# retrojetpacks/Gadget-Leicester

Hardware: AMD Instinct MI355X
Metric: particle-steps/sec (gravity+SPH) (higher is better)
Workload: dtype f64

## Files before the change

### gadget-leicester_amd/csrc/ghip_gravity.hip

```cpp
#include <cmath>

#include <hipcub/hipcub.hpp>

#include "ghip_walk.h"

__global__ void k_grav_finish(int nt, const int *__restrict__ tgt, const int *__restrict__ perm,
                              int n, double G, double comoving_fac, const double *__restrict__ pos,
                              const double *__restrict__ gravpm, double *__restrict__ oacc,
                              double *__restrict__ oldacc)
{
  int ti = blockIdx.x * blockDim.x + threadIdx.x;
  if(ti >= nt)
    return;
  int i = perm[tgt[ti]];
  double a0 = oacc[i], a1 = oacc[(size_t) n + i], a2 = oacc[2 * (size_t) n + i];
  if(comoving_fac != 0)
    {
      a0 += comoving_fac * pos[i];
      a1 += comoving_fac * pos[(size_t) n + i];
      a2 += comoving_fac * pos[2 * (size_t) n + i];
    }
  double b0 = a0, b1 = a1, b2 = a2;
  if(gravpm)
    {
// ... 537 lines not shown
{
  int per;
  ghip_shard_range(nt, ctx->shard_n, ctx->shard_rank, lo, cnt, &per);
}

struct WalkJob
{
  int walk;
  GravK k;
  WalkSeg sg;
  WalkPlan plan;
  PartialBufs pb;
  int nbuckets;
  unsigned long long *counter;
};

static int prepare_job(ghip_ctx *ctx, const ghip_grav_params *p, int walk, int nt, int slot,
                       WalkJob &J, hipStream_t plan_on = nullptr)
{
  hipStream_t ps = plan_on ? plan_on : ctx->stream;
  J.walk = walk;
  GCHK(prepare_tables(ctx, p, walk, J.k));
  walk_layout(ctx->dyn_use ? ctx->dyn.tree : ctx->gt, nt, J.sg, &J.nbuckets, walk == GHIP_WALK_EWALD);
  GCHK(build_plan(ctx, walk == GHIP_WALK_EWALD ? 1 : 0, J.nbuckets, J.sg.ns, J.plan, slot, ps));
  GCHK(ensure_partials(ctx, J.plan.nwaves, slot, J.pb));
  J.counter = ghip_cslot(ctx, walk == GHIP_WALK_EWALD ? GHIP_CK_EWALD : GHIP_CK_NEWTON);
  HIPCHK(hipMemsetAsync(J.counter, 0, GHIP_CKIND_U64 * 8, ps));
  return GHIP_OK;
}

static int run_walk(ghip_ctx *ctx, const WalkJob &J, int nt, const int *tgt, hipStream_t st)
{
  int evi = (J.walk == GHIP_WALK_EWALD) ? 4 : 2;
  ctx->plan_writer[J.walk == GHIP_WALK_EWALD ? 1 : 0] = st;
  HIPCHK(hipEventRecord(ctx->evp[evi], st));
  launch_walk_any(ctx, J.walk, ctx->dyn_use ? ctx->dyn.tree : ctx->gt, J.sg, J.nbuckets, nt, tgt, P<double>(ctx->sx),
                  P<double>(ctx->sy), P<double>(ctx->sz), P<double>(ctx->ssoft),
                  P<double>(ctx->soldacc), J.k, J.counter, J.plan, J.pb, st);
  HIPCHK(hipGetLastError());
  HIPCHK(hipEventRecord(ctx->evp[evi + 1], st));
  return GHIP_OK;
}

static int combine_walk(ghip_ctx *ctx, const WalkJob &J, int nt, const int *tgt, hipStream_t st)
{
  k_combine_grav<<<cdiv(nt, 256), 256, 0, st>>>(
    nt, J.plan, tgt, P<int>(ctx->gt.perm), J.pb.ax, J.pb.ay, J.pb.az, J.pb.cost, ctx->n,
    P<double>(ctx->f[GHIP_F_GRAVACCEL]), P<int>(ctx->f[GHIP_F_GRAVCOST]),
    J.walk == GHIP_WALK_EWALD ? 1 : 0, J.k.debug_steps);
  HIPCHK(hipGetLastError());
  return GHIP_OK;
}

static int pair_balance(ghip_ctx *ctx)
{
  if(!ctx->pc_ev[3][3])
    {
      for(int i = 0; i < 4; i++)
        for(int j = 0; j < 4; j++)
          if(!ctx->pc_ev[i][j])
            HIPCHK(hipEventCreate(&ctx->pc_ev[i][j]));
      return GHIP_OK;
    }
  for(int i = 0; i < 4; i++)
    {
      if(ctx->pc_cap[i] == 0)
        continue;
      hipEvent_t *e = ctx->pc_ev[i];
      if(hipEventQuery(e[1]) != hipSuccess || hipEventQuery(e[3]) != hipSuccess)
        {
          (void) hipGetLastError();
          continue;
        }
      float tn = 0, te = 0;
      if(hipEventElapsedTime(&tn, e[0], e[1]) == hipSuccess && hipEventElapsedTime(&te, e[2], e[3]) == hipSuccess)
        {
          const int k = ctx->pc_cap[i] > 8192 ? 1 : 0;
          const float fe = ctx->pc_hyd[i] ? 1.1f : 1.0f;
          const float c = tn > fe * te ? tn : fe * te;
          ctx->pc_cost[k] = c;
          ctx->pc_age[k] = 0;
        }
      else
        (void) hipGetLastError();
      ctx->pc_cap[i] = 0;
    }
  ctx->pc_age[0]++;
  ctx->pc_age[1]++;
  const int cur = ctx->pair_lds > 8192 ? 1 : 0, oth = cur ^ 1;
  if(ctx->pc_cost[cur] < 0)
    return GHIP_OK;
  int want = cur;
  const bool close = ctx->pc_cost[oth] > 0 && ctx->pc_cost[oth] < 1.1f * ctx->pc_cost[cur] &&
                     ctx->pc_cost[cur] < 1.1f * ctx->pc_cost[oth];
  if(ctx->pc_cost[oth] < 0 || ctx->pc_age[oth] > (close ? 16 : 64))
    want = oth;
  else if(ctx->pc_cost[oth] < ctx->pc_cost[cur])
    want = oth;
  ctx->pair_lds = want ? 10240 : 8192;
  static int dbg = -1;
  if(dbg < 0)
    dbg = getenv("GHIP_PAIR_DEBUG") ? 1 : 0;
  if(dbg)
    fprintf(stderr, "[pair_balance] cost 8K %.3f (age %d)  10K %.3f (age %d)  -> %d\n", ctx->pc_cost[0],
            ctx->pc_age[0], ctx->pc_cost[1], ctx->pc_age[1], ctx->pair_lds);
  return GHIP_OK;
}

int ghip_gravity_impl(ghip_ctx *ctx, const ghip_grav_params *p, int walk)
{
  if(!ctx->gt.built)
    return ghip_fail(ctx, GHIP_EINVAL, "ghip_gravity: call ghip_tree_build first");
  if(walk < 0 || walk > GHIP_WALK_NEWTON_EWALD)
    return ghip_fail(ctx, GHIP_EINVAL, "ghip_gravity: unknown walk %d", walk);
  const bool pair = (walk == GHIP_WALK_NEWTON_EWALD);
  if(pair && !p->periodic)
    return ghip_fail(ctx, GHIP_EINVAL, "ghip_gravity: the Newton+Ewald pair needs periodic = 1");
  if(ctx->tree_unverified)
    {
      ghip_ctx::GravCall c;
      c.p = *p;
      c.walk = walk;
      ctx->grav_log.push_back(c);
    }
  GCHK(ghip_build_target_lists(ctx));
  hipStream_t st = ctx->stream;
  int n = ctx->n;
  int lo, nt;
  shard_slice(ctx, ctx->nt_grav, &lo, &nt);
  ghip_stats &S = ctx->stats;
  if(walk == GHIP_WALK_EWALD || pair)
    S.ewald_interactions = 0;
  if(walk != GHIP_WALK_EWALD)
    {
      S.grav_interactions = 0;
      S.grav_targets = nt;
    }
  if(nt == 0 || n == 0)
    return GHIP_OK;
  const int *tgt = P<int>(ctx->tg_grav) + lo;
  WalkJob A, E;
  hipStream_t pn = (pair && ctx->plan_writer[0] == ctx->stream3) ? ctx->stream3 : nullptr;
  hipStream_t pe = (pair && ctx->plan_writer[1] == ctx->stream2) ? ctx->stream2 : nullptr;
  if(getenv("GHIP_PLAN_ON_MAIN"))
    pn = nullptr;
  GCHK(prepare_job(ctx, p, pair ? GHIP_WALK_NEWTON : walk, nt, 0, A, pn));
  if(pair)
    GCHK(prepare_job(ctx, p, GHIP_WALK_EWALD, nt, 1, E, pe));

  GCHK(ghip_gather_f64_lim(ctx, ctx->gt.n, P<int>(ctx->gt.perm), P<double>(ctx->f[GHIP_F_OLDACC]),
                           n, P<double>(ctx->soldacc)));
  if(!pair)
    {
      GCHK(run_walk(ctx, A, nt, tgt, st));
      return combine_walk(ctx, A, nt, tgt, st);
    }
  hipStream_t sN = ctx->stream3, sE = ctx->stream2;
  HIPCHK(hipEventRecord(ctx->evx[0], st));
// ... 220 lines not shown
```

### gadget-leicester_amd/csrc/ghip_internal.h

```cpp
#pragma once
#include <hip/hip_runtime.h>

#include <cstdint>
#include <cstdio>
#include <cstdlib>
#include <cstring>
#include <new>
#include <string>
#include <vector>

#include "../../include/ghip.h"
#include "ghip_count.h"

#define GHIP_BITS 21
#define GHIP_EN 64
#define GHIP_EW_NB ((GHIP_EN >> 1) + 1)
#define GHIP_EW_NKB (GHIP_EN / 3 + 1)
#define GHIP_EW_DOUBLES (GHIP_EW_NB * GHIP_EW_NB * GHIP_EW_NKB * 16)
static inline __host__ __device__ unsigned int ghip_ew_offset(int i, int j, int kb, int t)
{
  return (unsigned int) ((((i >> 1) * GHIP_EW_NB + (j >> 1)) * GHIP_EW_NKB + kb) * 16 +
                         ((i & 1) * 2 + (j & 1)) * 4 + t);
}
#define GHIP_NTAB 1000
// ... 172 lines not shown
  int du_sent = 0, du_recvd = 0;
  bool geom_kept = false;
  long long bytes_sent[16] = {0, 0, 0, 0, 0, 0, 0, 0, 0, 0, 0, 0, 0, 0, 0, 0};
  ghip_pm_params pm;
  DevBuf pm_all;
  int pmreg_grid = 0;
  ghip_pmnp_params pmnp;
  int pmnp_rc = 0;
  std::string pmnp_msg;
  ghip_pot_params pot;
  DevBuf pot_tgt;
  bool gt_is_pot = false;
  int pot_rc = 0;
  std::string pot_msg;
  ghip_dd_global_args gq;
  ghip_global_params gq_p;
  DevBuf gq_send, gq_all;
  ghip_dd_decomp_params dcp;
  DevBuf dc_own, dc_all;
  DevBuf dc_hist, dc_hist_all;
  int dc_level = 0, dc_bmax = 0, dc_shift = 0;
  int dc_rc = 0;
  std::string dc_msg;
  double dc_corner[3] = {0, 0, 0}, dc_center[3] = {0, 0, 0}, dc_len = 0;
};

static inline void ghip_dd_set_allgather(DDState &D, const void *send, size_t bytes, DevBuf *recv)
{
  D.x.kind = 1;
  D.x.send = send;
  D.x.bytes = bytes;
  D.x.recv = recv;
}

static inline void ghip_dd_set_alltoallv(DDState &D, const void *send, size_t recbytes,
                                         const int *scount, const int *soff, DevBuf *recv)
{
  D.x.kind = 2;
  D.x.send = send;
  D.x.bytes = recbytes;
  D.x.recv = recv;
  for(int r = 0; r < D.nranks; r++)
    {
      D.x.scount[r] = scount[r];
      D.x.soff[r] = soff[r];
    }
}

struct DevWords
{
  alignas(128) unsigned int pair_started;
  alignas(128) unsigned long long ghost_growth;
  unsigned long long timebin_hist[64];
  int sel_left;
  int list_count;
  int dust_partners;
  int gas_targets;
  int step_err;
  int pm_err;
  int tree_info[2][2];
};

struct alignas(64) PinnedWords
{
  TreeSizes sizes[2];
  int gas_mixed;
};

struct DynTree
{
  TreeDev tree;
  DevBuf ev, dp;
  DevBuf eh, cnt, fa;
  DevBuf kick;
  DevBuf kick_dv, kick_flag;
};

struct PmMesh
{
  int n = 0;
  void *fwd = nullptr, *inv = nullptr;
  DevBuf rho, k, force;
  struct Open
  {
    int n = 0;
    int table_n = 0;
    void *fwd = nullptr, *inv = nullptr;
    DevBuf rho, k, table, force, oct;
    Open() = default;
    Open(const Open &) = delete;
    Open &operator=(const Open &) = delete;
    ~Open();
  } open;
  PmMesh() = default;
  PmMesh(const PmMesh &) = delete;
  PmMesh &operator=(const PmMesh &) = delete;
  ~PmMesh();
};

struct ghip_ctx
{
  ghip_ctx() = default;
  ghip_ctx(const ghip_ctx &) = delete;
  ghip_ctx &operator=(const ghip_ctx &) = delete;
  ~ghip_ctx();

  int device = 0;
  hipStream_t stream = nullptr;
  std::string err;

  int n = 0, ngas = 0;
  DevBuf f[GHIP_F_COUNT];
  DevBuf stage, aosP, aosS;
  PinnedWords *pinned = nullptr;

  double corner[3] = {0, 0, 0}, center[3] = {0, 0, 0}, dlen = 0;
  double soft[6] = {0, 0, 0, 0, 0, 0};

  TreeDev gt;
  TreeDev st;
  DevBuf sx, sy, sz, ssoft, soldacc;
  DevBuf gp;
  DevBuf gq;
  DevBuf dleft, dright, drho, dnumngb, ddhsml, ddivv, drot, dflags, dtgt_a, dtgt_b, dhcur;
  DevBuf hpart;

  DevBuf act_host_idx;
  int nactive = -1;
  bool gas_mixed = false;
  int skip_massless = 0;
  bool massless_marked = false;
  bool gas_types_unknown = false;
  bool lists_dirty = true;
  bool gas_list_dirty = true;
  DevBuf tg_grav, tg_gas;
  int nt_grav = 0, nt_gas = 0;
  int shard_rank = 0, shard_n = 1;

  DevBuf tax, tay, taz, tcost;
  DevBuf tax2, tay2, taz2, tcost2, plan_nsub2, plan_woff2, plan_wave2, cubtmp2;
  hipStream_t stream2 = nullptr;
  hipStream_t stream3 = nullptr;
  bool adaptive_gravsoft = false;
  bool grav_pending = false;
  unsigned int *pair_started = nullptr;
  bool gas_pending = false;
  bool gas_wait_upload = false;
  hipEvent_t evx[4] = {};
  hipEvent_t evt[2] = {};
  DevBuf plan_steps[3][2], plan_nsub, plan_woff, plan_wave;
  int plan_nb[3] = {-1, -1, -1}, plan_ns[3] = {-1, -1, -1}, plan_cur[3] = {0, 0, 0};
// ... 1 lines not shown
  DevBuf cubtmp3;

  DevBuf ewtab;
  DevBuf ewbrick;
  double ew_box = 0;
  DevBuf srtab;
  bool srtab_ready = false;

  DevBuf cubtmp;
  PmMesh pm;
  ghip_pm_region pm_region = {};
  bool pm_region_set = false;
  DevBuf words;
  DevBuf cslots, rslots;
  ghip_stats stats;
  hipEvent_t ev[16] = {};
  DDState dd;
  DevBuf bh_swallow, bh_injected;
  DevBuf dust_heat;
  DevBuf dust_idx, dust_work, dust_pairs, dust_cub;
  DevBuf sfr_work, sfr_cub;
  int timestep_endrun = 0;
  bool iflags_on = false;
  ghip_integration_flags iflags = {};
  DevBuf kick_drag, kick_ddm, kick_newdens;
  bool has_drag = false, has_ddm = false, has_newdens = false;
  int kick_fields_n = -1, kick_fields_ngas = -1;

  bool visc_on = false;
  ghip_visc_params visc = {};
  DevBuf visc_alpha, visc_dtalpha;
  int visc_ngas = -1;
  long long visc_epoch = 0;

  bool async = false;
  bool tree_unverified = false;
  bool tree_async_ok = true;
  hipEvent_t ev_sizes = nullptr, ev_sizes_gas = nullptr;
  bool gas_unverified = false;
  bool gas_async = false;
  int build_gen = 0;
  bool sort_wide = false;
  bool in_recover = false;
  struct GravCall
  {
    ghip_grav_params p;
    int walk;
  };
  std::vector<GravCall> grav_log;
  std::vector<void *> host_pins;
  bool hydro_early = false;
  bool dyn_on = false, dyn_valid = false, dyn_use = false;
  DynTree dyn;
  int pair_lds = 10240;
  hipEvent_t pc_ev[4][4] = {};
  int pc_cap[4] = {0, 0, 0, 0};
  int pc_hyd[4] = {0, 0, 0, 0};
  int pc_head = 0;
  float pc_cost[2] = {-1.f, -1.f};
  int pc_age[2] = {0, 0};
  hipEvent_t ev_side = nullptr;

  std::vector<hipEvent_t> ev_ring;
  int ring_slots = 0, ring_cur = -1;
  hipEvent_t *evp = nullptr;
  long long run_steps = 0, run_syncs0 = 0, run_launches0 = 0, run_dens_iter = 0;
  long long n_syncs = 0;
  DevBuf pot;
  DevBuf pot_nint;
  int pot_n = -1;
  DevBuf potcorr;
  double potcorr_box = 0;
  DevBuf srpot;
  DevBuf gq_work;
};
#define GHIP_NEV 16

static inline hipError_t ghip_stream_sync(ghip_ctx *ctx, hipStream_t st)
{
  ctx->n_syncs++;
  return hipStreamSynchronize(st);
}
static inline hipError_t ghip_event_sync(ghip_ctx *ctx, hipEvent_t e)
{
  ctx->n_syncs++;
  return hipEventSynchronize(e);
}
long long ghip_launch_count(void);
int ghip_tree_verify(ghip_ctx *ctx);
int ghip_gas_verify(ghip_ctx *ctx);

int ghip_fail(ghip_ctx *ctx, int code, const char *fmt, ...);
#define GHIP_ERRW_PLAN 0
#define GHIP_ERRW_LET 1
#define GHIP_ERRW_TREE 2
#define GHIP_ERRW_PM 3
#define GHIP_ERRW_DRIFT 4
#define GHIP_ERRW_TIMESTEP 5
#define GHIP_ERRW_COUNT 8
int *ghip_errwords(void);
static inline int *ghip_errword(ghip_ctx *, int which) { return ghip_errwords() + which; }
int ghip_check_device_errors(ghip_ctx *ctx);
int ghip_join(ghip_ctx *ctx);
static inline int ghip_wg(const ghip_ctx *ctx) { return ctx->grav_pending ? 64 : 256; }
static inline int *ghip_gas_mixed_word(ghip_ctx *ctx) { return &ctx->pinned->gas_mixed; }
static inline DevWords *ghip_words(ghip_ctx *ctx) { return reinterpret_cast<DevWords *>(ctx->words.p); }
static inline unsigned long long *ghip_cslot(ghip_ctx *ctx, int kind)
{
  return reinterpret_cast<unsigned long long *>(ctx->cslots.p) + (size_t) kind * GHIP_CKIND_U64;
}
static inline unsigned long long *ghip_rslot(ghip_ctx *ctx, int kind)
{
  return reinterpret_cast<unsigned long long *>(ctx->rslots.p) + (size_t) kind * GHIP_CKIND_U64;
}
int ghip_read_slots(ghip_ctx *ctx, DevBuf &buf, unsigned long long out[GHIP_CK_COUNT][2]);
int ghip_mark_converted_gas(ghip_ctx *ctx);
int ghip_sink_buffers(ghip_ctx *ctx);
int ghip_unmark_massless_for_hydro(ghip_ctx *ctx);
int ghip_check_gas_types(ghip_ctx *ctx);
int ghip_dyn_capture(ghip_ctx *ctx);
int ghip_dyn_kick_recorded(ghip_ctx *ctx);
void ghip_dyn_release(ghip_ctx *ctx);
int ghip_fill_walk_records(ghip_ctx *ctx, TreeDev &t);
int ghip_gravity_finish_on(ghip_ctx *ctx, double G, int pmgrid, double comoving_fac, int all_shards,
                           hipStream_t st);
int ghip_join_pair(ghip_ctx *ctx);
int ghip_finish_gas_tree(ghip_ctx *ctx);
#define GHIP_JOIN(ctx)                          \
  do                                            \
    {                                           \
      int j_ = ghip_join(ctx);                  \
      if(j_ != GHIP_OK)                         \
        return j_;                              \
    }                                           \
  while(0)
void ghip_pm_release(ghip_ctx *ctx);
int ghip_pm_potential_add(ghip_ctx *ctx, const ghip_pm_params *p, double *pot);
int ghip_pm_potential_deposit(ghip_ctx *ctx, const ghip_pm_params *p);
int ghip_pm_potential_solve(ghip_ctx *ctx, const ghip_pm_params *p, int nranks, const double *all, double *pot);
int ghip_pmnp_potential_check(ghip_ctx *ctx, const ghip_grav_params *g, const ghip_pm_params *pm, const char *who);
int ghip_pmnp_potential_deposit(ghip_ctx *ctx, int pmgrid, int *outside);
int ghip_pmnp_potential_solve(ghip_ctx *ctx, int pmgrid, double G, int nranks, const double *all, double *pot);
size_t ghip_pmnp_block_bytes(int pmgrid);
const void *ghip_pmnp_block(ghip_ctx *ctx);
#define EXTENT_WORDS 16
int ghip_extent_pass(ghip_ctx *ctx, DevBuf &own, int use_work);
unsigned long long ghip_extent_reduce(const unsigned long long *all, int nranks, double xmin[3], double xmax[3],
                                      unsigned long long *ntot, int *bmin, int *bmax, int *bad);
#define EXTENT_ERR_POS 1ULL
#define EXTENT_ERR_WORK 2ULL
#define EXTENT_ERR_LOCAL 4ULL

#define HIPCHK(call)                                                                         \
  do                                                                                         \
    {                                                                                        \
      hipError_t e_ = (call);                                                                \
      if(e_ != hipSuccess)                                                                   \
// ... 123 lines not shown
```

### gadget-leicester_amd/csrc/ghip_sph.hip

```cpp

#include "ghip_ngb.h"
#include <cmath>

struct BucketBox
{
  double cx, cy, cz, ex, ey, ez, hmax;
};

__device__ __forceinline__ double d_first_lane_f64(double v)
{
  int lo = __builtin_amdgcn_readfirstlane(__double2loint(v));
  int hi = __builtin_amdgcn_readfirstlane(__double2hiint(v));
  return __hiloint2double(hi, lo);
}

__device__ __forceinline__ BucketBox d_bucket_box(bool valid, double px, double py, double pz,
                                                  double h, const BoxK b)
{
  BucketBox B;
  B.cx = d_first_lane_f64(px);
  B.cy = d_first_lane_f64(py);
  B.cz = d_first_lane_f64(pz);
  B.ex = d_wave_max_f64(valid ? fabs(d_wrap(px - B.cx, b)) : 0.0);
  B.ey = d_wave_max_f64(valid ? fabs(d_wrap(py - B.cy, b)) : 0.0);
// ... 541 lines not shown
      if(b < nblk)
        blockcnt[b] = run + incl - c;
      run += __shfl(incl, 63, 64);
    }
  if(threadIdx.x == 0)
    *total = run;
}

__global__ void __launch_bounds__(64) k_sel_scatter(int n, const int *__restrict__ in,
                                                    const int *__restrict__ flags,
                                                    const int *__restrict__ blockoff,
                                                    int *__restrict__ out)
{
  const int base = blockIdx.x * SEL_BLOCK;
  int off = blockoff[blockIdx.x];
  const unsigned long long below = (1ull << threadIdx.x) - 1ull;
  for(int j = 0; j < SEL_ITEMS; j++)
    {
      const int a = base + j * 64 + threadIdx.x;
      const bool keep = a < n && flags[a] != 0;
      const unsigned long long m = __ballot(keep);
      if(keep)
        out[off + __popcll(m & below)] = in[a];
      off += __popcll(m);
    }
}

int ghip_density_impl(ghip_ctx *ctx, const ghip_dens_params *p)
{
  GCHK(ghip_tree_verify(ctx));
  GCHK(ghip_finish_gas_tree(ctx));
  if(ctx->gas_wait_upload)
    return ghip_fail(ctx, GHIP_EINVAL, "ghip_density: ghip_upload_aos_particles was not followed by "
                     "ghip_upload_aos_gas");
  GCHK(ghip_gas_verify(ctx));
  if(!ctx->st.built)
    return ghip_fail(ctx, GHIP_EINVAL, "ghip_density: call ghip_tree_build first");
  GCHK(ghip_build_target_lists(ctx));
  ghip_stats &S = ctx->stats;
  S.dens_neighbours = 0;
  S.dens_target_evals = 0;
  S.dens_iterations = 0;
  int ng = ctx->ngas, n = ctx->n;
  int lo, nt;
  shard_slice(ctx, ctx->nt_gas, &lo, &nt);
  if(ng == 0 || nt == 0)
    return GHIP_OK;
  hipStream_t st = ctx->stream;
  TreeDev &t = ctx->st;
  GCHK(dens_alloc(ctx));
  double *hcur = P<double>(ctx->dhcur);
  unsigned long long *counter = ghip_cslot(ctx, GHIP_CK_DENS);
  unsigned long long *racc = ghip_rslot(ctx, GHIP_CK_DENS);
  int *dnum = &ghip_words(ctx)->sel_left;
  HIPCHK(hipMemsetAsync(counter, 0, GHIP_CKIND_U64 * 8, st));
  HIPCHK(hipEventRecord(ctx->evp[6], st));

  int *cur = P<int>(ctx->dtgt_a), *nxt = P<int>(ctx->dtgt_b);
  HIPCHK(hipMemcpyAsync(cur, P<int>(ctx->tg_gas) + lo, (size_t) nt * 4, hipMemcpyDeviceToDevice,
                        st));
  k_dens_init<<<cdiv(nt, ghip_wg(ctx)), ghip_wg(ctx), 0, st>>>(nt, cur, P<double>(ctx->gp), hcur,
                                             P<double>(ctx->dleft), P<double>(ctx->dright));
  BoxK b = make_box(p->BoxSize, p->periodic);
  DensFin F = {p->DesNumNgb, p->MaxNumNgbDeviation, p->MinGasHsml, p->Ti_Current,
               p->Timebase_interval};
  int maxiter = p->MaxIter > 0 ? p->MaxIter : 150;
  int ncur = nt, iter = 0;
  GCHK(ghip_ensure(ctx, ctx->cubtmp, ((size_t) cdiv(nt, SEL_BLOCK) + 2) * 4));
  int *seloff = P<int>(ctx->cubtmp);

  while(ncur > 0)
    {
      const int tgw = ghip_sph_tg();
      const int nbk = (ncur + tgw - 1) / tgw;
      int nsub = (ghip_sph_target_waves() + nbk - 1) / nbk;
      nsub = nsub < 1 ? 1 : (nsub > GHIP_MAXSUB ? GHIP_MAXSUB : nsub);
      SPH_LAUNCH(k_density, tgw, (nbk * nsub + 7) & ~7, st, P<TreeSizes>(t.dsz), P<SphNode>(t.mq), P<double>(ctx->gp), ncur,
                 nsub, cur, hcur, b, P<double>(ctx->drho), P<double>(ctx->dnumngb),
                 P<double>(ctx->ddhsml), P<double>(ctx->ddivv), P<double>(ctx->drot), counter, racc,
                 ghip_sph_xcd(), nbk * nsub);
      k_dens_finalize<<<cdiv(ncur, ghip_wg(ctx)), ghip_wg(ctx), 0, st>>>(
        ncur, nsub, cur, P<int>(t.perm), n, ng, F, P<double>(ctx->drho), P<double>(ctx->dnumngb),
        P<double>(ctx->ddhsml), P<double>(ctx->ddivv), P<double>(ctx->drot), hcur,
        P<double>(ctx->dleft), P<double>(ctx->dright), P<double>(ctx->f[GHIP_F_ENTROPY]),
        P<double>(ctx->f[GHIP_F_DTENTROPY]), P<int>(ctx->f[GHIP_F_TIMEBIN]),
        P<int>(ctx->f[GHIP_F_TI_BEGSTEP]), P<double>(ctx->gp), P<double>(ctx->gq),
        P<double>(ctx->f[GHIP_F_HSML]), P<double>(ctx->f[GHIP_F_NUMNGB]),
        P<double>(ctx->f[GHIP_F_DENSITY]), P<double>(ctx->f[GHIP_F_DHSMLFAC]),
        P<double>(ctx->f[GHIP_F_DIVVEL]), P<double>(ctx->f[GHIP_F_CURLVEL]),
        P<double>(ctx->f[GHIP_F_PRESSURE]), P<int>(ctx->dflags));
      HIPCHK(hipGetLastError());
      S.dens_target_evals += ncur;
      const int nblk = cdiv(ncur, SEL_BLOCK);
      k_sel_count<<<nblk, 64, 0, st>>>(ncur, P<int>(ctx->dflags), seloff);
      k_sel_scan<<<1, 64, 0, st>>>(nblk, seloff, dnum);
      int left = 0;
      HIPCHK(hipMemcpyAsync(&left, dnum, 4, hipMemcpyDeviceToHost, st));
      HIPCHK(ghip_stream_sync(ctx, st));
      GCHK(ghip_check_device_errors(ctx));
      if(left > 0)
        {
          k_sel_scatter<<<nblk, 64, 0, st>>>(ncur, cur, P<int>(ctx->dflags), seloff, nxt);
          HIPCHK(hipGetLastError());
        }
      ncur = left;
      int *tmp = cur;
      cur = nxt;
      nxt = tmp;
      if(ncur > 0)
        {
          iter++;
          if(iter > maxiter)
            return ghip_fail(ctx, GHIP_ENOCONV,
                             "density: %d particles not converged after %d h-iterations "
                             "(reference: endrun(1155), density.c:669-674)", ncur, maxiter);
        }
    }
  HIPCHK(hipEventRecord(ctx->evp[7], st));
  S.dens_iterations = iter;
  return GHIP_OK;
}

extern "C" int ghip_density(ghip_ctx *ctx, const ghip_dens_params *p)
{
  if(!ctx || !p)
    return GHIP_EINVAL;
  return ghip_density_impl(ctx, p);
}

extern "C" int ghip_update_hmax(ghip_ctx *ctx)
{
  if(!ctx)
    return GHIP_EINVAL;
  GCHK(ghip_tree_verify(ctx));
  GCHK(ghip_finish_gas_tree(ctx));
  GCHK(ghip_gas_verify(ctx));
  if(!ctx->st.built)
    return ghip_fail(ctx, GHIP_EINVAL, "ghip_update_hmax: no tree");
  return ghip_gastree_refresh_hmax(ctx);
}

extern "C" int ghip_density_evaluate(ghip_ctx *ctx, const ghip_dens_params *p, int target,
                                     double h, double out7[7])
{
  if(ctx)
    GHIP_JOIN(ctx);
  if(!ctx || !p || !out7)
    return GHIP_EINVAL;
  GCHK(ghip_finish_gas_tree(ctx));
  if(!ctx->st.built)
    return ghip_fail(ctx, GHIP_EINVAL, "ghip_density_evaluate: no tree");
// ... 698 lines not shown
```

### gadget-leicester_amd/csrc/ghip_tree.hip

```cpp
#include <hipcub/hipcub.hpp>

#include "ghip_internal.h"
#include "ghip_keys.h"

__global__ void k_morton_from_pos(int n, const double *__restrict__ x, const double *__restrict__ y,
                                  const double *__restrict__ z, double cx, double cy, double cz,
                                  double fac, unsigned long long *__restrict__ key,
                                  int *__restrict__ idx)
{
  int i = blockIdx.x * blockDim.x + threadIdx.x;
  if(i >= n)
    return;
  int ix = (int) ((x[i] - cx) * fac);
  int iy = (int) ((y[i] - cy) * fac);
  int iz = (int) ((z[i] - cz) * fac);
  key[i] = d_morton21(ix, iy, iz);
  idx[i] = i;
}

__global__ void k_morton_from_ints(int n, const int *__restrict__ x, const int *__restrict__ y,
                                   const int *__restrict__ z, int bits,
                                   unsigned long long *__restrict__ key)
{
  int i = blockIdx.x * blockDim.x + threadIdx.x;
// ... 437 lines not shown
                             const double *__restrict__ vy, const double *__restrict__ vz,
                             const double *__restrict__ h, const double *__restrict__ pres,
                             const double *__restrict__ rho, const double *__restrict__ dhf,
                             const double *__restrict__ divv, const double *__restrict__ curl,
                             const int *__restrict__ timebin, double *__restrict__ gp,
                             double *__restrict__ gq)
{
  int s = blockIdx.x * blockDim.x + threadIdx.x;
  if(s >= ng)
    return;
  int i = perm[s];
  double *r = gp + (size_t) 8 * s;
  r[0] = x[i];
  r[1] = y[i];
  r[2] = z[i];
  r[3] = m[i];
  r[4] = vx[i];
  r[5] = vy[i];
  r[6] = vz[i];
  r[7] = h[i];
  double *q = gq + (size_t) 8 * s;
  int tb = timebin[i];
  q[0] = pres[i];
  q[1] = rho[i];
  q[2] = dhf[i];
  q[3] = divv[i];
  q[4] = curl[i];
  q[5] = (double) (tb ? (1 << tb) : 0);
  q[6] = 0;
  q[7] = 0;
}

__global__ void k_gather_f64_lim(int n, const int *__restrict__ perm, const double *__restrict__ src,
                                 int limit, double *__restrict__ dst)
{
  int s = blockIdx.x * blockDim.x + threadIdx.x;
  if(s < n)
    {
      int i = perm[s];
      dst[s] = i < limit ? src[i] : 0.0;
    }
}

int ghip_gather_f64_lim(ghip_ctx *ctx, int n, const int *perm, const double *src, int limit,
                        double *dst)
{
  if(n <= 0)
    return GHIP_OK;
  k_gather_f64_lim<<<cdiv(n, 256), 256, 0, ctx->stream>>>(n, perm, src, limit, dst);
  HIPCHK(hipGetLastError());
  return GHIP_OK;
}

int ghip_gather_f64(ghip_ctx *ctx, int n, const int *perm, const double *src, double *dst)
{
  if(n <= 0)
    return GHIP_OK;
  k_gather_f64<<<cdiv(n, 256), 256, 0, ctx->stream>>>(n, perm, src, dst);
  HIPCHK(hipGetLastError());
  return GHIP_OK;
}

__global__ void k_mark_active(int nact, const int *__restrict__ act, const int *__restrict__ iperm,
                              int limit, int *__restrict__ flags)
{
  int a = blockIdx.x * blockDim.x + threadIdx.x;
  if(a >= nact)
    return;
  int i = act[a];
  if(i >= 0 && i < limit)
    flags[iperm[i]] = 1;
}

__global__ void k_key_hi(int n, int shift, const unsigned long long *__restrict__ key,
                         unsigned int *__restrict__ hi)
{
  int i = blockIdx.x * blockDim.x + threadIdx.x;
  if(i < n)
    hi[i] = (unsigned int) (key[i] >> shift);
}

__global__ void k_gather_keys(int n, const int *__restrict__ perm,
                              const unsigned long long *__restrict__ key,
                              unsigned long long *__restrict__ skey)
{
  int s = blockIdx.x * blockDim.x + threadIdx.x;
  if(s < n)
    skey[s] = key[perm[s]];
}

__global__ void k_fix_runs(int n, int maxrun, unsigned long long *__restrict__ skey,
                           int *__restrict__ perm, int *__restrict__ longest)
{
  int s = blockIdx.x * blockDim.x + threadIdx.x;
  if(s >= n)
    return;
  unsigned int h = (unsigned int) (skey[s] >> 31);
  if(s > 0 && (unsigned int) (skey[s - 1] >> 31) == h)
    return;
  int e = s + 1;
  while(e < n && (unsigned int) (skey[e] >> 31) == h)
    e++;
  int len = e - s;
  if(len == 1)
    return;
  if(len > maxrun)
// ... 1054 lines not shown
    flags[s] = 0;
}

int ghip_mark_converted_gas(ghip_ctx *ctx)
{
  TreeDev &t = ctx->st;
  if((!ctx->gas_mixed && !ctx->skip_massless) || t.n == 0)
    return GHIP_OK;
  const int wg = ghip_wg(ctx);
  k_mark_converted<<<cdiv(t.n, wg), wg, 0, ctx->stream>>>(t.n, ctx->ngas, ctx->skip_massless ? 1 : 0,
                                                          P<int>(t.perm), P<int>(ctx->f[GHIP_F_TYPE]),
                                                          P<double>(ctx->gp));
  HIPCHK(hipGetLastError());
  ctx->massless_marked = ctx->skip_massless != 0;
  return GHIP_OK;
}

__global__ void k_unmark_massless(int nsrc, int ngas, const int *__restrict__ perm, const int *__restrict__ type,
                                  double *__restrict__ gp)
{
  int s = blockIdx.x * blockDim.x + threadIdx.x;
  if(s >= nsrc)
    return;
  const int i = perm[s];
  if(gp[(size_t) 8 * s + 3] < 0 && (i >= ngas || type[i] == 0))
    gp[(size_t) 8 * s + 3] = 0.0;
}

int ghip_unmark_massless_for_hydro(ghip_ctx *ctx)
{
  TreeDev &t = ctx->st;
  if(!ctx->massless_marked || ctx->skip_massless != 1 || t.n == 0)
    return GHIP_OK;
  const int wg = ghip_wg(ctx);
  k_unmark_massless<<<cdiv(t.n, wg), wg, 0, ctx->stream>>>(t.n, ctx->ngas, P<int>(t.perm),
                                                           P<int>(ctx->f[GHIP_F_TYPE]), P<double>(ctx->gp));
  HIPCHK(hipGetLastError());
  ctx->massless_marked = false;
  return GHIP_OK;
}

static int make_list(ghip_ctx *ctx, TreeDev &t, int host_limit, DevBuf &list, int *count)
{
  hipStream_t st = ctx->stream;
  int n = t.n;
  *count = 0;
  if(n == 0)
    return GHIP_OK;
  GCHK(ghip_ensure(ctx, list, (size_t) n * 4));
  const bool imports = n > host_limit;
  const bool mixed = (&t == &ctx->st) && ctx->gas_mixed;
  if(ctx->nactive < 0 && !imports && !mixed)
    {
      HIPCHK(hipMemcpyAsync(list.p, t.phorder.p, (size_t) n * 4, hipMemcpyDeviceToDevice, st));
      *count = n;
      return GHIP_OK;
    }
  if(ctx->nactive == 0)
    return GHIP_OK;
  GCHK(ghip_ensure(ctx, ctx->dflags, (size_t) n * 4));
  GCHK(ghip_ensure(ctx, ctx->dtgt_a, (size_t) n * 4 + 16));
  if(ctx->nactive < 0)
    k_flag_local<<<cdiv(n, 256), 256, 0, st>>>(n, host_limit, P<int>(t.perm), P<int>(ctx->dflags));
  else
    {
      HIPCHK(hipMemsetAsync(ctx->dflags.p, 0, (size_t) n * 4, st));
      k_mark_active<<<cdiv(ctx->nactive, 256), 256, 0, st>>>(ctx->nactive, P<int>(ctx->act_host_idx),
                                                              P<int>(t.iperm), host_limit,
                                                              P<int>(ctx->dflags));
    }
  if(mixed)
    k_unflag_converted<<<cdiv(n, 256), 256, 0, st>>>(n, host_limit, P<int>(t.perm), P<int>(ctx->f[GHIP_F_TYPE]),
                                                    P<int>(ctx->dflags));
  k_gather_i32<<<cdiv(n, 256), 256, 0, st>>>(n, P<int>(t.phorder), P<int>(ctx->dflags),
                                             P<int>(ctx->dtgt_a));
  HIPCHK(hipGetLastError());
  int *dnum = &ghip_words(ctx)->list_count;
  size_t tb = 0;
  HIPCHK(hipcub::DeviceSelect::Flagged(nullptr, tb, P<int>(t.phorder), P<int>(ctx->dtgt_a),
                                       P<int>(list), dnum, n, st));
  GCHK(cub_tmp(ctx, tb));
  HIPCHK(hipcub::DeviceSelect::Flagged(ctx->cubtmp.p, tb, P<int>(t.phorder),
                                       P<int>(ctx->dtgt_a), P<int>(list), dnum, n, st));
  HIPCHK(hipMemcpyAsync(count, dnum, 4, hipMemcpyDeviceToHost, st));
  HIPCHK(ghip_stream_sync(ctx, st));
  return GHIP_OK;
}

struct ShardLoT
{
  int lo[GHIP_MAXRANKS + 1];
};

__global__ void k_shard_permute(int nt, int nranks, ShardLoT L, const int *__restrict__ src,
                                int *__restrict__ dst)
{
  int j = blockIdx.x * blockDim.x + threadIdx.x;
  if(j >= nt)
    return;
  int r = 0;
  while(r + 1 < nranks && j >= L.lo[r + 1])
    r++;
  int a = j - L.lo[r];
  int gb = (a >> 6) * nranks + r;
  dst[j] = src[gb * 64 + (a & 63)];
}

// ... 43 lines not shown
```

### gadget-leicester_amd/csrc/ghip_walk.h

```cpp
#pragma once
#include "ghip_internal.h"
#include "ghip_count.h"

#ifndef GHIP_WALK_WAVES
#define GHIP_WALK_WAVES 8
#endif
#ifndef GHIP_WALK_OPT
#define GHIP_WALK_OPT 15
#endif


struct GravK
{
  double theta;
  double errtol;
  double boxsize, boxhalf;
  int periodic, unequal;
  int debug_steps;
  int xcd_remap;
  double rcut, rcut2, asmthfac;
  double fac_intp;
  double k1875;
};

// ... 39 lines not shown
__device__ __forceinline__ void d_load2(const T *__restrict__ base, int ea, v16i &A, int eb, v16i &B)
{
  const unsigned int oa = d_rec_off(ea), ob = d_rec_off(eb);
  asm volatile("s_load_dwordx16 %0, %2, %3\n\ts_load_dwordx16 %1, %2, %4\n\ts_waitcnt lgkmcnt(0)"
               : "=&s"(A), "=&s"(B)
               : "s"(base), "s"(oa), "s"(ob)
               : "memory");
}
template <class T>
__device__ __forceinline__ void d_touch_next(const T *__restrict__ base, unsigned int off, int &scratch)
{
  asm volatile("s_load_dword %0, %1, %2 offset:0x40" : "=s"(scratch) : "s"(base), "s"(off) : "memory");
}
template <class T>
__device__ __forceinline__ void d_touch(const T *__restrict__ base, int e, int &scratch)
{
  const unsigned int off = d_rec_off(e);
  asm volatile("s_load_dword %0, %1, %2" : "=s"(scratch) : "s"(base), "s"(off) : "memory");
}
template <class T>
__device__ __forceinline__ void d_load1_touch(const T *__restrict__ base, unsigned int off, v16i &R,
                                              int &s1, int &s2)
{
  asm volatile("s_load_dwordx16 %0, %3, %4\n\ts_waitcnt lgkmcnt(0)"
               : "=s"(R), "+s"(s1), "+s"(s2)
               : "s"(base), "s"(off)
               : "memory");
}
__device__ __forceinline__ void d_drain_touch(int &s1, int &s2)
{
  asm volatile("s_waitcnt lgkmcnt(0) ; drain-touches" : "+s"(s1), "+s"(s2) : : "memory");
}

__device__ __forceinline__ double d_rsqrt(double x)
{
  double y = __builtin_amdgcn_rsq(x);
  double t = x * y;
  double e = fma(-t, y, 1.0);
  double p = fma(0.375, e, 0.5);
  return fma(y * e, p, y);
}

__device__ __forceinline__ double d_mass_over_r3(double mass, double x, double k15 = 1.5,
                                                 double k1875 = 1.875)
{
  double y = __builtin_amdgcn_rsq(x);
  double y2 = y * y;
  double e = fma(-x, y2, 1.0);
  double p = fma(k1875, e, k15);
  double c = (mass * y) * y2;
  return fma(c * e, p, c);
}

__device__ __forceinline__ double d_grav_fac(double mass, double r2, double h, double h2,
                                             double &r_out)
{
  if(r2 >= h2)
    {
      double rinv = d_rsqrt(r2);
      r_out = r2 * rinv;
      return mass * rinv * rinv * rinv;
    }
  double r = sqrt(r2);
  r_out = r;
  double h_inv = 1.0 / h;
  double h3_inv = h_inv * h_inv * h_inv;
  double u = r * h_inv;
  if(u < 0.5)
    return mass * h3_inv * (10.666666666667 + u * u * (32.0 * u - 38.4));
  return mass * h3_inv *
         (21.333333333333 - 48.0 * u + 38.4 * u * u - 10.666666666667 * u * u * u -
          0.066666666667 / (u * u * u));
}

template <bool BRICK>
__device__ __forceinline__ void d_ewald_interp(const double *__restrict__ tab, double fac_intp,
                                               double dx, double dy, double dz, double &fx,
                                               double &fy, double &fz)
{
  const int E1 = GHIP_EN + 1;
  const double sx = dx < 0 ? 1.0 : -1.0, sy = dy < 0 ? 1.0 : -1.0, sz = dz < 0 ? 1.0 : -1.0;
  dx = fabs(dx);
  dy = fabs(dy);
  dz = fabs(dz);
  double u = dx * fac_intp;
  int i = (int) u;
  if(i >= GHIP_EN)
    i = GHIP_EN - 1;
  u -= i;
  double v = dy * fac_intp;
  int j = (int) v;
  if(j >= GHIP_EN)
    j = GHIP_EN - 1;
  v -= j;
  double w = dz * fac_intp;
  int k = (int) w;
  if(k >= GHIP_EN)
    k = GHIP_EN - 1;
  w -= k;
  double f1 = (1 - u) * (1 - v) * (1 - w), f2 = (1 - u) * (1 - v) * (w);
  double f3 = (1 - u) * (v) * (1 - w), f4 = (1 - u) * (v) * (w);
  double f5 = (u) * (1 - v) * (1 - w), f6 = (u) * (1 - v) * (w);
  double f7 = (u) * (v) * (1 - w), f8 = (u) * (v) * (w);
  EwPair x00, x01, x10, x11, y00, y01, y10, y11, z00, z01, z10, z11;
  if(!BRICK)
    {
      const unsigned int ui = (unsigned int) i, uj = (unsigned int) j, uk = (unsigned int) k;
      const unsigned int R1 = E1 * 8u, R2 = E1 * E1 * 8u;
      const unsigned int ox = (ui * E1 + uj) * R1 + uk * 8u;
      const unsigned int oy = (uj * E1 + ui) * R1 + uk * 8u;
      const unsigned int oz = (uk * E1 + uj) * R1 + ui * 8u;
      const unsigned int ox2 = ox + R2, oy2 = oy + R2, oz2 = oz + R2;
      const char *tb = reinterpret_cast<const char *>(tab);
#define EW_LD(off, imm) d_ldpair(reinterpret_cast<const double *>(tb + (size_t) (off) + (imm)))
      x00 = EW_LD(ox, 0), x01 = EW_LD(ox, R1), x10 = EW_LD(ox2, 0), x11 = EW_LD(ox2, R1);
      y00 = EW_LD(oy, 0), y01 = EW_LD(oy, R1), y10 = EW_LD(oy2, 0), y11 = EW_LD(oy2, R1);
      z00 = EW_LD(oz, 0), z01 = EW_LD(oz, R1), z10 = EW_LD(oz2, 0), z11 = EW_LD(oz2, R1);
#undef EW_LD
    }
  else
    {
      const unsigned int SA = GHIP_EW_NB * GHIP_EW_NKB * 128, SB = GHIP_EW_NKB * 128;
      const unsigned int ai = (i >> 1) * SA + (i & 1) * 64, ai1 = ((i + 1) >> 1) * SA + ((i + 1) & 1) * 64;
      const unsigned int aj = (j >> 1) * SA + (j & 1) * 64, aj1 = ((j + 1) >> 1) * SA + ((j + 1) & 1) * 64;
      const unsigned int ak = (k >> 1) * SA + (k & 1) * 64, ak1 = ((k + 1) >> 1) * SA + ((k + 1) & 1) * 64;
// ... 315 lines not shown
                                                const float *__restrict__ srtab,
                                                const double *__restrict__ ewtab, bool valid,
                                                WalkLane &W, int &my_skip, unsigned int &steps)
{
  while(c.kseg < sg.ns)
    {
      const int s0 = __builtin_amdgcn_readfirstlane(sg.start[c.kseg]);
      c.s1 = __builtin_amdgcn_readfirstlane(sg.start[c.kseg + 1]);
      my_skip = valid ? 0 : 0x7fffffff;
      const int na = __builtin_amdgcn_readfirstlane(sg.nanc[c.kseg]);
      for(int a = 0; a < na; a++)
        {
          int ea = __builtin_amdgcn_readfirstlane(sg.anc[c.kseg * GHIP_MAXANC + a]);
          v16i H;
          d_load1(hot, ea, H);
          d_walk_element<MODE, PERIODIC, UNEQUAL, false, REL>(ea, H, cold, p, srtab, ewtab, W, my_skip);
          steps++;
        }
      int first = d_wave_min_i32(my_skip);
      c.e = __builtin_amdgcn_readfirstlane(first > s0 ? first : s0);
      if(c.e < c.s1)
        return true;
      c.kseg += stride;
    }
  return false;
}

template <int MODE, bool PERIODIC, bool UNEQUAL, bool REL>
__device__ __forceinline__ void d_walk_run(const WalkSeg &sg, int sub, const WalkHot *__restrict__ hot,
                                           const WalkCold *__restrict__ cold, const GravK &p,
                                           const float *__restrict__ srtab,
                                           const double *__restrict__ ewtab, bool valid, WalkLane &W,
                                           unsigned int &steps)
{
  if(MODE != GHIP_WALK_EWALD)
    {
      SegCursor A;
      int skipA = 0;
      A.kseg = sub;
      const int stride = sg.nsub;
      bool liveA = d_enter_segment<MODE, PERIODIC, UNEQUAL, REL>(A, stride, sg, hot, cold, p, srtab,
                                                            ewtab, valid, W, skipA, steps);
      int t1 = 0, t2 = 0;
      while(liveA)
        {
          v16i HA;
          const unsigned int offA = d_rec_off(A.e);
          d_load1_touch(hot, offA, HA, t1, t2);
          d_touch_next(hot, offA, t1);
          d_touch(hot, d_lo32(HA, 6), t2);
          steps++;
          A.e = __builtin_amdgcn_readfirstlane(
            d_walk_element<MODE, PERIODIC, UNEQUAL, true, REL>(A.e, HA, cold, p, srtab, ewtab, W, skipA));
          if(A.e >= A.s1)
            {
              d_drain_touch(t1, t2);
              A.kseg += stride;
              liveA = d_enter_segment<MODE, PERIODIC, UNEQUAL, REL>(A, stride, sg, hot, cold, p, srtab,
                                                               ewtab, valid, W, skipA, steps);
            }
        }
      d_drain_touch(t1, t2);
    }
  else
    {
      SegCursor A, B;
      int skipA = 0, skipB = 0;
      A.kseg = sub;
      B.kseg = sub + sg.nsub;
      const int stride = 2 * sg.nsub;
      bool liveA = d_enter_segment<MODE, PERIODIC, UNEQUAL, REL>(A, stride, sg, hot, cold, p, srtab, ewtab, valid,
                                                   W, skipA, steps);
      bool liveB = d_enter_segment<MODE, PERIODIC, UNEQUAL, REL>(B, stride, sg, hot, cold, p, srtab, ewtab, valid,
                                                   W, skipB, steps);
      while(liveA && liveB)
        {
          v16i HA, HB;
          d_load2(hot, A.e, HA, B.e, HB);
          steps += 2;
          A.e = __builtin_amdgcn_readfirstlane(
            d_walk_element<MODE, PERIODIC, UNEQUAL, true, REL>(A.e, HA, cold, p, srtab, ewtab, W, skipA));
          B.e = __builtin_amdgcn_readfirstlane(
            d_walk_element<MODE, PERIODIC, UNEQUAL, true, REL>(B.e, HB, cold, p, srtab, ewtab, W, skipB));
          if(A.e >= A.s1)
            {
              A.kseg += stride;
              liveA = d_enter_segment<MODE, PERIODIC, UNEQUAL, REL>(A, stride, sg, hot, cold, p, srtab, ewtab,
                                                      valid, W, skipA, steps);
            }
          if(B.e >= B.s1)
            {
              B.kseg += stride;
              liveB = d_enter_segment<MODE, PERIODIC, UNEQUAL, REL>(B, stride, sg, hot, cold, p, srtab, ewtab,
                                                      valid, W, skipB, steps);
            }
        }
      if(liveB)
        {
          A = B;
          skipA = skipB;
          liveA = true;
        }
      while(liveA)
        {
          v16i HA;
          d_load1(hot, A.e, HA);
          steps++;
// ... 325 lines not shown
```

Baseline: 81.60 million.

## Add third pair LDS setting, pinned sel counter, copy kernels, cold softening path

The pair LDS autotuner now picks among three dynamic-LDS caps (6K/8K/10K) instead of two, and skips probing settings that still have pending measurements. The selection-left counter moves into pinned host memory so the host reads it after a stream sync without a separate device-to-host copy. Device-to-device memcpys are replaced by a small copy kernel. The softened-gravity branch of the walk is split into a noinline cold function and the segment-exit branch is marked unlikely, to reduce register pressure and code size in the hot walk loop. Together these touch several unrelated costs, and each carries its own risk, such as a call overhead when the softening branch is taken.

New measurement: 85.51 million, median of 6. +4.8%, better.

```diff
diff --git a/gadget-leicester_amd/csrc/ghip_gravity.hip b/gadget-leicester_amd/csrc/ghip_gravity.hip
--- a/gadget-leicester_amd/csrc/ghip_gravity.hip
+++ b/gadget-leicester_amd/csrc/ghip_gravity.hip
@@ -613,6 +613,17 @@
   return GHIP_OK;
 }
 
+static const int pair_caps[GHIP_PAIR_NSET] = {GHIP_PAIR_LDS(6), GHIP_PAIR_LDS(5), GHIP_PAIR_LDS(4)};
+
+static int pair_setting(int lds)
+{
+  int k = 0;
+  for(int j = 1; j < GHIP_PAIR_NSET; j++)
+    if(lds >= pair_caps[j])
+      k = j;
+  return k;
+}
+
 static int pair_balance(ghip_ctx *ctx)
 {
   if(!ctx->pc_ev[3][3])
@@ -623,6 +634,7 @@
             HIPCHK(hipEventCreate(&ctx->pc_ev[i][j]));
       return GHIP_OK;
     }
+  bool pending[GHIP_PAIR_NSET] = {};
   for(int i = 0; i < 4; i++)
     {
       if(ctx->pc_cap[i] == 0)
@@ -631,12 +643,13 @@
       if(hipEventQuery(e[1]) != hipSuccess || hipEventQuery(e[3]) != hipSuccess)
         {
           (void) hipGetLastError();
+          pending[pair_setting(ctx->pc_cap[i])] = true;
           continue;
         }
       float tn = 0, te = 0;
       if(hipEventElapsedTime(&tn, e[0], e[1]) == hipSuccess && hipEventElapsedTime(&te, e[2], e[3]) == hipSuccess)
         {
-          const int k = ctx->pc_cap[i] > 8192 ? 1 : 0;
+          const int k = pair_setting(ctx->pc_cap[i]);
           const float fe = ctx->pc_hyd[i] ? 1.1f : 1.0f;
           const float c = tn > fe * te ? tn : fe * te;
           ctx->pc_cost[k] = c;
@@ -646,25 +659,40 @@
         (void) hipGetLastError();
       ctx->pc_cap[i] = 0;
     }
-  ctx->pc_age[0]++;
-  ctx->pc_age[1]++;
-  const int cur = ctx->pair_lds > 8192 ? 1 : 0, oth = cur ^ 1;
-  if(ctx->pc_cost[cur] < 0)
+  for(int k = 0; k < GHIP_PAIR_NSET; k++)
+    ctx->pc_age[k]++;
+  const int cur = pair_setting(ctx->pair_lds);
+  const float *cost = ctx->pc_cost;
+  if(cost[cur] < 0)
     return GHIP_OK;
-  int want = cur;
-  const bool close = ctx->pc_cost[oth] > 0 && ctx->pc_cost[oth] < 1.1f * ctx->pc_cost[cur] &&
-                     ctx->pc_cost[cur] < 1.1f * ctx->pc_cost[oth];
-  if(ctx->pc_cost[oth] < 0 || ctx->pc_age[oth] > (close ? 16 : 64))
-    want = oth;
-  else if(ctx->pc_cost[oth] < ctx->pc_cost[cur])
-    want = oth;
-  ctx->pair_lds = want ? 10240 : 8192;
+  int want = cur, probe = -1;
+  for(int k = 0; k < GHIP_PAIR_NSET; k++)
+    {
+      if(k == cur || pending[k])
+        continue;
+      const bool close = cost[k] > 0 && cost[k] < 1.1f * cost[cur] && cost[cur] < 1.1f * cost[k];
+      if(cost[k] < 0 || ctx->pc_age[k] > (close ? 16 : 64))
+        {
+          if(probe < 0 || (cost[k] < 0 && cost[probe] >= 0) ||
+             ((cost[k] < 0) == (cost[probe] < 0) && ctx->pc_age[k] > ctx->pc_age[probe]))
+            probe = k;
+        }
+      else if(cost[k] < cost[want])
+        want = k;
+    }
+  if(probe >= 0)
+    want = probe;
+  ctx->pair_lds = pair_caps[want];
   static int dbg = -1;
   if(dbg < 0)
     dbg = getenv("GHIP_PAIR_DEBUG") ? 1 : 0;
   if(dbg)
-    fprintf(stderr, "[pair_balance] cost 8K %.3f (age %d)  10K %.3f (age %d)  -> %d\n", ctx->pc_cost[0],
-            ctx->pc_age[0], ctx->pc_cost[1], ctx->pc_age[1], ctx->pair_lds);
+    {
+      fprintf(stderr, "[pair_balance] cost");
+      for(int k = 0; k < GHIP_PAIR_NSET; k++)
+        fprintf(stderr, " %dK %.3f (age %d)", pair_caps[k] >> 10, cost[k], ctx->pc_age[k]);
+      fprintf(stderr, "  -> %d\n", ctx->pair_lds);
+    }
   return GHIP_OK;
 }
 
diff --git a/gadget-leicester_amd/csrc/ghip_internal.h b/gadget-leicester_amd/csrc/ghip_internal.h
--- a/gadget-leicester_amd/csrc/ghip_internal.h
+++ b/gadget-leicester_amd/csrc/ghip_internal.h
@@ -248,7 +248,6 @@
   alignas(128) unsigned int pair_started;
   alignas(128) unsigned long long ghost_growth;
   unsigned long long timebin_hist[64];
-  int sel_left;
   int list_count;
   int dust_partners;
   int gas_targets;
@@ -261,6 +260,7 @@
 {
   TreeSizes sizes[2];
   int gas_mixed;
+  int sel_left;
 };
 
 struct DynTree
@@ -293,6 +293,13 @@
   PmMesh &operator=(const PmMesh &) = delete;
   ~PmMesh();
 };
+
+#define GHIP_LDS_PER_CU 163840
+#define GHIP_LDS_GRANULE 2048
+#define GHIP_PAIR_LDS(W) ((GHIP_LDS_PER_CU / (4 * (W))) / GHIP_LDS_GRANULE * GHIP_LDS_GRANULE)
+#define GHIP_PAIR_NSET 3
+static_assert(GHIP_PAIR_LDS(4) == 10240 && GHIP_PAIR_LDS(5) == 8192 && GHIP_PAIR_LDS(6) == 6144,
+              "dynamic-LDS caps of the pair");
 
 struct ghip_ctx
 {
@@ -400,13 +407,13 @@
   bool hydro_early = false;
   bool dyn_on = false, dyn_valid = false, dyn_use = false;
   DynTree dyn;
-  int pair_lds = 10240;
+  int pair_lds = GHIP_PAIR_LDS(5);
   hipEvent_t pc_ev[4][4] = {};
   int pc_cap[4] = {0, 0, 0, 0};
   int pc_hyd[4] = {0, 0, 0, 0};
   int pc_head = 0;
-  float pc_cost[2] = {-1.f, -1.f};
-  int pc_age[2] = {0, 0};
+  float pc_cost[GHIP_PAIR_NSET] = {-1.f, -1.f, -1.f};
+  int pc_age[GHIP_PAIR_NSET] = {0, 0, 0};
   hipEvent_t ev_side = nullptr;
 
   std::vector<hipEvent_t> ev_ring;
@@ -451,6 +458,7 @@
 int ghip_check_device_errors(ghip_ctx *ctx);
 int ghip_join(ghip_ctx *ctx);
 static inline int ghip_wg(const ghip_ctx *ctx) { return ctx->grav_pending ? 64 : 256; }
+int ghip_copy_i32(ghip_ctx *ctx, int *dst, const int *src, size_t n);
 static inline int *ghip_gas_mixed_word(ghip_ctx *ctx) { return &ctx->pinned->gas_mixed; }
 static inline DevWords *ghip_words(ghip_ctx *ctx) { return reinterpret_cast<DevWords *>(ctx->words.p); }
 static inline unsigned long long *ghip_cslot(ghip_ctx *ctx, int kind)
diff --git a/gadget-leicester_amd/csrc/ghip_sph.hip b/gadget-leicester_amd/csrc/ghip_sph.hip
--- a/gadget-leicester_amd/csrc/ghip_sph.hip
+++ b/gadget-leicester_amd/csrc/ghip_sph.hip
@@ -617,13 +617,12 @@
   double *hcur = P<double>(ctx->dhcur);
   unsigned long long *counter = ghip_cslot(ctx, GHIP_CK_DENS);
   unsigned long long *racc = ghip_rslot(ctx, GHIP_CK_DENS);
-  int *dnum = &ghip_words(ctx)->sel_left;
+  int *dnum = &ctx->pinned->sel_left;
   HIPCHK(hipMemsetAsync(counter, 0, GHIP_CKIND_U64 * 8, st));
   HIPCHK(hipEventRecord(ctx->evp[6], st));
 
   int *cur = P<int>(ctx->dtgt_a), *nxt = P<int>(ctx->dtgt_b);
-  HIPCHK(hipMemcpyAsync(cur, P<int>(ctx->tg_gas) + lo, (size_t) nt * 4, hipMemcpyDeviceToDevice,
-                        st));
+  GCHK(ghip_copy_i32(ctx, cur, P<int>(ctx->tg_gas) + lo, (size_t) nt));
   k_dens_init<<<cdiv(nt, ghip_wg(ctx)), ghip_wg(ctx), 0, st>>>(nt, cur, P<double>(ctx->gp), hcur,
                                              P<double>(ctx->dleft), P<double>(ctx->dright));
   BoxK b = make_box(p->BoxSize, p->periodic);
@@ -659,9 +658,8 @@
       const int nblk = cdiv(ncur, SEL_BLOCK);
       k_sel_count<<<nblk, 64, 0, st>>>(ncur, P<int>(ctx->dflags), seloff);
       k_sel_scan<<<1, 64, 0, st>>>(nblk, seloff, dnum);
-      int left = 0;
-      HIPCHK(hipMemcpyAsync(&left, dnum, 4, hipMemcpyDeviceToHost, st));
       HIPCHK(ghip_stream_sync(ctx, st));
+      const int left = *reinterpret_cast<const volatile int *>(dnum);
       GCHK(ghip_check_device_errors(ctx));
       if(left > 0)
         {
diff --git a/gadget-leicester_amd/csrc/ghip_tree.hip b/gadget-leicester_amd/csrc/ghip_tree.hip
--- a/gadget-leicester_amd/csrc/ghip_tree.hip
+++ b/gadget-leicester_amd/csrc/ghip_tree.hip
@@ -513,6 +513,27 @@
   return GHIP_OK;
 }
 
+__global__ void __launch_bounds__(64) k_copy_i32(size_t n, const int *__restrict__ src, int *__restrict__ dst)
+{
+  const size_t base = (size_t) blockIdx.x * 1024 + threadIdx.x;
+#pragma unroll 4
+  for(int j = 0; j < 16; j++)
+    {
+      const size_t a = base + (size_t) j * 64;
+      if(a < n)
+        dst[a] = src[a];
+    }
+}
+
+int ghip_copy_i32(ghip_ctx *ctx, int *dst, const int *src, size_t n)
+{
+  if(n == 0)
+    return GHIP_OK;
+  k_copy_i32<<<(unsigned int) ((n + 1023) / 1024), 64, 0, ctx->stream>>>(n, src, dst);
+  HIPCHK(hipGetLastError());
+  return GHIP_OK;
+}
+
 int ghip_gather_f64(ghip_ctx *ctx, int n, const int *perm, const double *src, double *dst)
 {
   if(n <= 0)
@@ -1673,7 +1694,7 @@
   const bool mixed = (&t == &ctx->st) && ctx->gas_mixed;
   if(ctx->nactive < 0 && !imports && !mixed)
     {
-      HIPCHK(hipMemcpyAsync(list.p, t.phorder.p, (size_t) n * 4, hipMemcpyDeviceToDevice, st));
+      GCHK(ghip_copy_i32(ctx, P<int>(list), P<int>(t.phorder), (size_t) n));
       *count = n;
       return GHIP_OK;
     }
diff --git a/gadget-leicester_amd/csrc/ghip_walk.h b/gadget-leicester_amd/csrc/ghip_walk.h
--- a/gadget-leicester_amd/csrc/ghip_walk.h
+++ b/gadget-leicester_amd/csrc/ghip_walk.h
@@ -115,25 +115,40 @@
   return fma(c * e, p, c);
 }
 
-__device__ __forceinline__ double d_grav_fac(double mass, double r2, double h, double h2,
-                                             double &r_out)
-{
-  if(r2 >= h2)
-    {
-      double rinv = d_rsqrt(r2);
-      r_out = r2 * rinv;
-      return mass * rinv * rinv * rinv;
-    }
+struct SoftFac
+{
+  double fac, r;
+};
+static __device__ __attribute__((noinline, cold)) SoftFac d_grav_fac_inside(double mass, double r2,
+                                                                            double h)
+{
+  SoftFac o;
   double r = sqrt(r2);
-  r_out = r;
+  o.r = r;
   double h_inv = 1.0 / h;
   double h3_inv = h_inv * h_inv * h_inv;
   double u = r * h_inv;
   if(u < 0.5)
-    return mass * h3_inv * (10.666666666667 + u * u * (32.0 * u - 38.4));
-  return mass * h3_inv *
-         (21.333333333333 - 48.0 * u + 38.4 * u * u - 10.666666666667 * u * u * u -
-          0.066666666667 / (u * u * u));
+    o.fac = mass * h3_inv * (10.666666666667 + u * u * (32.0 * u - 38.4));
+  else
+    o.fac = mass * h3_inv *
+            (21.333333333333 - 48.0 * u + 38.4 * u * u - 10.666666666667 * u * u * u -
+             0.066666666667 / (u * u * u));
+  return o;
+}
+
+__device__ __forceinline__ double d_grav_fac(double mass, double r2, double h, double h2,
+                                             double &r_out)
+{
+  if(r2 >= h2)
+    {
+      double rinv = d_rsqrt(r2);
+      r_out = r2 * rinv;
+      return mass * rinv * rinv * rinv;
+    }
+  const SoftFac s = d_grav_fac_inside(mass, r2, h);
+  r_out = s.r;
+  return s.fac;
 }
 
 template <bool BRICK>
@@ -555,7 +570,7 @@
           steps++;
           A.e = __builtin_amdgcn_readfirstlane(
             d_walk_element<MODE, PERIODIC, UNEQUAL, true, REL>(A.e, HA, cold, p, srtab, ewtab, W, skipA));
-          if(A.e >= A.s1)
+          if(__builtin_expect(A.e >= A.s1, 0))
             {
               d_drain_touch(t1, t2);
               A.kseg += stride;
```
